# tobifinn/torch-assimilate

Hardware: AMD Instinct MI355X
Metric: local analyses/sec (LETKF, 40-member) (higher is better)
Workload: dtype f32

## Files before the change

include/mia_letkf.h:

```cpp
#ifndef MIA_LETKF_H
#define MIA_LETKF_H

#include <stddef.h>
#include <stdint.h>

#ifdef __cplusplus
extern "C" {
#endif

#define MIA_VERSION 100

#define MIA_OK 0
#define MIA_ERR_NULL (-1)
#define MIA_ERR_SIZE (-2)
#define MIA_ERR_UNSUPPORTED (-3)
#define MIA_ERR_WORKSPACE (-4)
#define MIA_ERR_ALIGN (-5)
#define MIA_ERR_COMM (-6)
#define MIA_ERR_ARG (-7)

#define MIA_FLAG_OVERFLOW 1
#define MIA_FLAG_NOCONV 2
#define MIA_FLAG_NONFINITE 4
#define MIA_FLAG_RETRY 8
// ... 355 lines not shown
                               const double* rec, int64_t P,
                               const int32_t* nbr_cnt, const int32_t* nbr_idx, const double* nbr_w, int p_cap, int p_max,
                               double epsilon, double* W_out, int32_t* flags, int32_t* retry_count, void* stream);
int mia_lienks_update_wide_f64_cover(int k, int p_max, int64_t n_points, int64_t P);
int mia_lienks_update_stream_f64(const double* W_in, int64_t w_stride, int k, int64_t g0, int64_t g1,
                                 const double* rec, int64_t P,
                                 const int32_t* nbr_cnt, const int32_t* nbr_idx, const double* nbr_w, int p_cap, int p_max,
                                 double epsilon, double* W_out, int32_t* flags, int32_t* retry_count, void* stream);
int mia_lienks_update_stream_f64_cover(int k, int p_max, int64_t n_points, int64_t P);

int mia_obs_space_uncorr_f32(const float* hx, int64_t ldh, const float* y, const float* var, int k, int64_t P,
                             float* Yb_opt, int64_t ldy, float* d_opt, float* rec_opt, void* stream);
int mia_obs_space_uncorr_f64(const double* hx, int64_t ldh, const double* y, const double* var, int k, int64_t P,
                             double* Yb_opt, int64_t ldy, double* d_opt, double* rec_opt, void* stream);
int mia_obs_space_corr_workspace_bytes(int k, int64_t P, int elem_bytes, size_t* bytes);
int mia_obs_space_corr_f32(const float* hx, int64_t ldh, const float* y, const float* cov, int k, int64_t P,
                           float* Yb_opt, int64_t ldy, float* d_opt, float* rec_opt, int32_t* info_opt,
                           void* ws, size_t ws_bytes, void* stream);
int mia_obs_space_corr_f64(const double* hx, int64_t ldh, const double* y, const double* cov, int k, int64_t P,
                           double* Yb_opt, int64_t ldy, double* d_opt, double* rec_opt, int32_t* info_opt,
                           void* ws, size_t ws_bytes, void* stream);

typedef struct mia_comm mia_comm_t;
typedef int (*mia_allgather_fn)(void* ctx, const void* send, void* recv, size_t bytes_per_rank, void* stream);
typedef int (*mia_allreduce_max_i32_fn)(void* ctx, int32_t* buf, int n, void* stream);
int mia_comm_load(const char* rccl_library_path );
int mia_comm_unique_id(void* id128);
int mia_comm_create(const void* id128, int rank, int world, mia_comm_t** comm);
int mia_comm_create_partition(int rank, int world, mia_comm_t** out);
int mia_comm_create_custom(int rank, int world, mia_allgather_fn allgather, mia_allreduce_max_i32_fn allreduce_max,
                           void* ctx, mia_comm_t** comm);
int mia_letkf_step_submit(const float* X, int64_t G, int m, int k, const float* Yb, const float* d, int64_t P,
                          const double* grid_xyz, const double* obs_xyz, int n_coord, const int32_t* coord_group,
                          const double* gc_c, int n_r, double gc_eps, float inf_factor, float gamma, int method,
                          int p_max_assumed, mia_comm_t* comm, int n_chunks, int phase, float* Xa, int32_t* flags,
                          int32_t* counters, void* ws, size_t ws_bytes, void* stream, void* comm_stream, void* prep_stream,
                          int step_flags, int32_t* host8, void* after_stream, void* on_stream, void** done_event,
                          void* time_start_event, void* time_stop_event, void** job_out);
int mia_letkf_step_join(void* job);
typedef struct mia_step_args {
  const float* X; int64_t G; int32_t m, k; const float* Yb; const float* d; int64_t P;
  const double* grid_xyz; const double* obs_xyz; int32_t n_coord; int32_t coord_group[MIA_MAX_COORD];
  double gc_c[MIA_MAX_RADII]; int32_t n_r; double gc_eps; float inf_factor, gamma; int32_t method, p_max_assumed;
  mia_comm_t* comm; int32_t n_chunks, phase; float* Xa; int32_t* flags; int32_t* counters; void* ws; size_t ws_bytes;
  void* stream; void* comm_stream; void* prep_stream; int32_t step_flags; int32_t* host8; void* after_stream; void* on_stream;
  void** done_event; void* time_start_event; void* time_stop_event;
  void* caller_stream; void** in_event;
  double period[MIA_MAX_COORD];
} mia_step_args_t;
int mia_letkf_step_submit_args(const mia_step_args_t* a, void** job_out);
int mia_letkf_sharded_step_periodic_f32(const float* X, int64_t G, int m, int k, const float* Yb, const float* d, int64_t P,
                                        const double* grid_xyz, const double* obs_xyz, int n_coord, const int32_t* coord_group,
                                        const double* period, const double* gc_c, int n_r, double gc_eps, float inf_factor,
                                        float gamma, int method, int p_max_assumed, mia_comm_t* comm, int n_chunks, int phase,
                                        float* Xa, int32_t* flags, int32_t* counters, void* ws, size_t ws_bytes, void* stream,
                                        void* comm_stream, void* prep_stream, int step_flags);
int mia_letkf_step_run_args(const mia_step_args_t* a, int32_t* out8);
int mia_letkf_step_collect(void* job, void** done_event, const int32_t* host8, void* consumer_stream, int consumer_stream_valid,
                           int32_t* out8);
int mia_timing_event_acquire(void** event);
int mia_timing_event_release(void* event);
int mia_timing_event_elapsed_ms(void* start_event, void* stop_event, float* ms);
int mia_letkf_step_drain(void);
int mia_letkf_step_readback(const int32_t* counters, int32_t* host8, void* after_stream, void* on_stream, void** done_event);
int mia_event_synchronize(void* event);
int mia_stream_wait_event(void* stream, void* event);
int mia_stream_wait_stream(void* dst_stream, void* src_stream, void** event_io);
int mia_event_destroy(void* event);
int mia_letkf_step_launch_stats(double* prep_us, double* rest_us, long long* steps);
int mia_comm_set_place_stream(mia_comm_t* comm, void* stream);
int mia_comm_peer_alloc(mia_comm_t* comm, size_t result_bytes, int n_slots, void* ipc_handles_out);
int mia_comm_peer_open(mia_comm_t* comm, const void* all_handles);
int mia_comm_peer_attach(mia_comm_t* comm, int peer, void* const* result_bufs, void* sync_area);
int mia_comm_peer_wait_bound(mia_comm_t* comm, int log2_polls);
void* mia_comm_peer_buffer(mia_comm_t* comm, int slot);
void* mia_comm_peer_sync_area(mia_comm_t* comm);
int mia_comm_peer_exchange(mia_comm_t* comm, int slot, int rows, int64_t G, int64_t b0, int64_t b1, int32_t* counters,
                           void* stream);
int mia_comm_peer_rewait(mia_comm_t* comm, int slot, int32_t* counters, void* stream);
int mia_comm_destroy(mia_comm_t* comm);
const char* mia_comm_last_error(void);
int mia_letkf_sharded_step_workspace_bytes(int64_t G, int m, int k, int64_t P, int n_coord, int world,
                                           int n_chunks, int p_max_assumed, size_t* bytes);
int mia_letkf_step_workspace_release(void* ws);
int mia_debug_step_trace(long long* out, int max_steps);
int mia_letkf_sharded_step_f32(const float* X , int64_t G, int m, int k,
                               const float* Yb , const float* d , int64_t P,
                               const double* grid_xyz , const double* obs_xyz ,
                               int n_coord, const int32_t* coord_group , const double* gc_c ,
                               int n_r, double gc_eps, float inf_factor, float gamma, int method,
                               int p_max_assumed, mia_comm_t* comm, int n_chunks, int phase,
                               float* Xa , int32_t* flags, int32_t* counters,
                               void* ws, size_t ws_bytes, void* stream, void* comm_stream);

#define MIA_STEP_NO_JOIN 1
#define MIA_STEP_WS_CLEAN 4
#define MIA_STEP_TILE_EXTRA(n) (((n) & 7) << 4)
#define MIA_STEP_FRESH_BOX 0x400
#define MIA_STEP_SCAN_INDEX 0x800
#define MIA_STEP_REUSE_LISTS 0x1000
#define MIA_STEP_KEEP_LISTS 0x4000
#define MIA_STEP_NO_GATHER 0x2000
#define MIA_STEP_NO_TILE_LISTS 8
int mia_letkf_sharded_step_streams_f32(const float* X, int64_t G, int m, int k,
                                       const float* Yb, const float* d, int64_t P,
                                       const double* grid_xyz, const double* obs_xyz,
                                       int n_coord, const int32_t* coord_group , const double* gc_c ,
                                       int n_r, double gc_eps, float inf_factor, float gamma, int method,
                                       int p_max_assumed, mia_comm_t* comm, int n_chunks, int phase,
                                       float* Xa, int32_t* flags, int32_t* counters,
                                       void* ws, size_t ws_bytes, void* stream, void* comm_stream,
                                       void* prep_stream, int step_flags);

int mia_letkf_step_timing_events(void* start_event, void* stop_event);

#ifdef __cplusplus
}
#endif
#endif
```

torch-assimilate_amd/_cabi.py:

```python
import ctypes as C
import os

from ._build import LIB_PATH

_lib = None

i32, i64, f32, f64, vp, sz = C.c_int, C.c_int64, C.c_float, C.c_double, C.c_void_p, C.c_size_t


class KernelOp(C.Structure):
    _fields_ = [("op", C.c_int32), ("reserved", C.c_int32), ("value", C.c_double)]


_LISTS = [vp, vp, vp, i32, i32]
_SHARD = [vp, i64, i32, i32, i64, i64, vp, i64] + _LISTS


def _analysis_entry(f):
    return (_SHARD + [f, f, vp, i64, i64, vp, vp, vp], i32)


def _analysis_redo(f):
    return (_SHARD + [f, f, vp, i64, i64, vp, vp], i32)

# ... 82 lines not shown
    "mia_letkf_localize_tiles_periodic_f64": ([i32, vp, i64, i64, vp, i64, i32, C.POINTER(C.c_int32), C.POINTER(f64),
                                               C.POINTER(f64), i32, f64, i32, i32, vp, sz, vp, vp, sz, vp], i32),
    "mia_letkf_analysis_matfun_fused_f32": ([vp, i64, i32, i32, i64, i64, vp, i64, vp, i32, C.POINTER(C.c_int32),
                                             C.POINTER(f64), i32, f64, vp, sz, i32, f32, f32, vp, i64, i64, vp, vp, vp,
                                             vp], i32),
    "mia_letkf_tile_lists_bytes": ([i64, i32, i32, C.POINTER(sz)], i32),
    "mia_letkf_localize_tiles_f64": ([i32, vp, i64, i64, vp, i64, i32, C.POINTER(C.c_int32), C.POINTER(f64), i32, f64,
                                      i32, i32, vp, sz, vp, vp, sz, vp], i32),
    "mia_letkf_split_record_bytes": ([i32, C.POINTER(sz)], i32),
    "mia_letkf_pack_split_f32": ([vp, vp, i32, i64, vp, vp], i32),
    "mia_letkf_analysis_tiles_f32": ([vp, i64, i32, i32, i64, i64, vp, i64, vp, i32, i32, f32, vp, i64, i64, vp, vp, vp], i32),
    "mia_letkf_tiles_cover": ([i32, i32, i32, i32, i64, i64, i64, i64, f32], i32),
    "mia_lketkf_rbf_analysis_tiles_f32": ([vp, i64, i32, i32, i64, i64, vp, vp, i64, vp, i32, i32, f32, f32, vp, i64, i64,
                                           vp, vp, vp], i32),
    "mia_letkf_weights_tiles_f32": ([vp, i64, i32, i32, i64, i64, vp, i64, vp, i32, i32, f32, vp, i64, i64, vp, vp, vp, vp], i32),
    "mia_letkf_analysis_retry_f32": _analysis_redo(f32),
    "mia_lketkf_rbf_analysis_f32": ([vp, i64, i32, i32, i64, i64, vp, vp, i64, vp, vp, vp, i32, i32, f32, f32,
                                     vp, i64, i64, vp, vp, vp, sz, vp], i32),
    "mia_lketkf_rbf_analysis_f64": ([vp, i64, i32, i32, i64, i64, vp, vp, i64, vp, vp, vp, i32, i32, f64, f64,
                                     vp, i64, i64, vp, vp, vp, sz, vp], i32),
    "mia_etkf_workspace_bytes": ([i32, i64, i32, C.POINTER(sz)], i32),
    "mia_etkf_weights_f32": ([vp, vp, i32, i64, f32, vp, vp, vp, sz, vp], i32),
    "mia_etkf_weights_f64": ([vp, vp, i32, i64, f64, vp, vp, vp, sz, vp], i32),
    "mia_ketkf_workspace_bytes": ([i32, i64, i32, C.POINTER(sz)], i32),
    "mia_ketkf_weights_f32": ([vp, vp, i32, i64, f32, C.POINTER(KernelOp), i32, vp, vp, vp, sz, vp], i32),
    "mia_ketkf_weights_f64": ([vp, vp, i32, i64, f64, C.POINTER(KernelOp), i32, vp, vp, vp, sz, vp], i32),
    "mia_apply_weights_f32": ([vp, i64, i32, i32, i64, i64, vp, vp, i64, i64, vp], i32),
    "mia_apply_weights_f64": ([vp, i64, i32, i32, i64, i64, vp, vp, i64, i64, vp], i32),
    "mia_apply_f64_cover": ([i32, i32, i64, i64, i64], i32),
    "mia_apply_local_f64_cover": ([i32, i32, i64, i64, i64], i32),
    "mia_apply_local_weights_f32": ([vp, i64, i32, i32, i64, i64, vp, vp, i64, i64, vp], i32),
    "mia_apply_local_weights_f64": ([vp, i64, i32, i32, i64, i64, vp, vp, i64, i64, vp], i32),
    "mia_lienks_update_f32": ([vp, i64, i32, i64, i64, vp, i64, vp, vp, vp, i32, i32, f32, f32, vp, vp, vp], i32),
    "mia_lienks_update_f64": ([vp, i64, i32, i64, i64, vp, i64, vp, vp, vp, i32, i32, f64, f64, vp, vp, vp], i32),
    "mia_lienks_update_matfun_f32": _ienks_tile_entry(f32),
    "mia_lienks_update_retry_f32": ([vp, i64, i32, i64, i64, vp, i64, vp, vp, vp, i32, i32, f32, f32, vp, vp, vp], i32),
    "mia_lienks_update_matfun_f64": _ienks_tile_entry(f64),
    "mia_lienks_update_retry_f64": ([vp, i64, i32, i64, i64, vp, i64, vp, vp, vp, i32, i32, f64, f64, vp, vp, vp], i32),
    "mia_lienks_update_f64_cover": _COVER4,
    "mia_lienks_update_wide_f64": _ienks_tile_entry(f64),
    "mia_lienks_update_wide_f64_cover": _COVER4,
    "mia_lienks_update_stream_f64": _ienks_tile_entry(f64),
    "mia_lienks_update_stream_f64_cover": _COVER4,
    "mia_obs_space_uncorr_f32": ([vp, i64, vp, vp, i32, i64, vp, i64, vp, vp, vp], i32),
    "mia_obs_space_uncorr_f64": ([vp, i64, vp, vp, i32, i64, vp, i64, vp, vp, vp], i32),
    "mia_obs_space_corr_workspace_bytes": ([i32, i64, i32, C.POINTER(sz)], i32),
    "mia_obs_space_corr_f32": ([vp, i64, vp, vp, i32, i64, vp, i64, vp, vp, vp, vp, sz, vp], i32),
    "mia_obs_space_corr_f64": ([vp, i64, vp, vp, i32, i64, vp, i64, vp, vp, vp, vp, sz, vp], i32),
    "mia_comm_load": ([C.c_char_p], i32),
    "mia_comm_unique_id": ([vp], i32),
    "mia_comm_create": ([vp, i32, i32, C.POINTER(vp)], i32),
    "mia_comm_create_partition": ([i32, i32, C.POINTER(vp)], i32),
    "mia_comm_create_custom": ([i32, i32, vp, vp, vp, C.POINTER(vp)], i32),
    "mia_comm_set_place_stream": ([vp, vp], i32),
    "mia_letkf_step_submit": ([vp, i64, i32, i32, vp, vp, i64, vp, vp, i32, C.POINTER(C.c_int32), C.POINTER(f64), i32, f64,
                               f32, f32, i32, i32, vp, i32, i32, vp, vp, vp, vp, sz, vp, vp, vp, i32,
                               vp, vp, vp, C.POINTER(vp), vp, vp, C.POINTER(vp)], i32),
    "mia_letkf_step_submit_args": ([vp, vp], i32),
    "mia_letkf_step_run_args": ([vp, vp], i32),
    "mia_letkf_step_collect": ([vp, vp, vp, vp, i32, vp], i32),
    "mia_timing_event_acquire": ([C.POINTER(vp)], i32),
    "mia_timing_event_release": ([vp], i32),
    "mia_timing_event_elapsed_ms": ([vp, vp, C.POINTER(C.c_float)], i32),
    "mia_letkf_step_join": ([vp], i32),
    "mia_debug_step_trace": ([C.POINTER(C.c_longlong), i32], i32),
    "mia_letkf_step_drain": ([], i32),
    "mia_letkf_step_readback": ([vp, vp, vp, vp, C.POINTER(vp)], i32),
    "mia_event_synchronize": ([vp], i32),
    "mia_stream_wait_event": ([vp, vp], i32),
    "mia_stream_wait_stream": ([vp, vp, C.POINTER(vp)], i32),
    "mia_event_destroy": ([vp], i32),
    "mia_letkf_step_launch_stats": ([C.POINTER(C.c_double), C.POINTER(C.c_double), C.POINTER(C.c_longlong)], i32),
    "mia_comm_peer_alloc": ([vp, sz, i32, vp], i32),
    "mia_comm_peer_open": ([vp, vp], i32),
    "mia_comm_peer_attach": ([vp, i32, C.POINTER(vp), vp], i32),
    "mia_comm_peer_wait_bound": ([vp, i32], i32),
    "mia_comm_peer_buffer": ([vp, i32], vp),
    "mia_comm_peer_sync_area": ([vp], vp),
    "mia_comm_peer_exchange": ([vp, i32, i32, i64, i64, i64, vp, vp], i32),
    "mia_comm_peer_rewait": ([vp, i32, vp, vp], i32),
    "mia_comm_destroy": ([vp], i32),
    "mia_comm_last_error": ([], C.c_char_p),
    "mia_letkf_sharded_step_workspace_bytes": ([i64, i32, i32, i64, i32, i32, i32, i32, C.POINTER(sz)], i32),
    "mia_letkf_step_workspace_release": ([vp], i32),
    "mia_letkf_sharded_step_f32": ([vp, i64, i32, i32, vp, vp, i64, vp, vp, i32, C.POINTER(C.c_int32), C.POINTER(f64),
                                    i32, f64, f32, f32, i32, i32, vp, i32, i32, vp, vp, vp, vp, sz, vp, vp], i32),
    "mia_letkf_step_timing_events": ([vp, vp], i32),
    "mia_letkf_sharded_step_streams_f32": ([vp, i64, i32, i32, vp, vp, i64, vp, vp, i32, C.POINTER(C.c_int32),
                                            C.POINTER(f64), i32, f64, f32, f32, i32, i32, vp, i32, i32, vp, vp, vp, vp,
                                            sz, vp, vp, vp, i32], i32),
    "mia_letkf_sharded_step_periodic_f32": ([vp, i64, i32, i32, vp, vp, i64, vp, vp, i32, C.POINTER(C.c_int32), C.POINTER(f64),
                                             C.POINTER(f64), i32, f64, f32, f32, i32, i32, vp, i32, i32, vp, vp, vp, vp,
                                             sz, vp, vp, vp, i32], i32),
}
EXPORTED_SYMBOLS = tuple(_PROTOS)
ALLGATHER_FN = C.CFUNCTYPE(C.c_int, vp, vp, vp, sz, vp)
ALLREDUCE_MAX_I32_FN = C.CFUNCTYPE(C.c_int, vp, vp, C.c_int, vp)


class MiaError(RuntimeError):
    status = None


def lib():
    global _lib
    if _lib is None:
        if not os.path.exists(LIB_PATH):
            raise MiaError(
                "HIP extension %s not found: run `python -c \"import __graft_entry__ as g; g.build()\"` "
                "(there is no CPU fallback for the LETKF hot path)" % LIB_PATH)
        import torch
        h = C.CDLL(LIB_PATH)
        for name, (args, res) in _PROTOS.items():
            fn = getattr(h, name)
            fn.argtypes, fn.restype = args, res
        _lib = h
    return _lib


def set_option(name: str, value: int) -> int:
    old = C.c_int(0)
    check(lib().mia_get_option(name.encode(), C.byref(old)), "mia_get_option(%s)" % name)
    check(lib().mia_set_option(name.encode(), int(value)), "mia_set_option(%s)" % name)
    return old.value


class StepArgs(C.Structure):
    _fields_ = [("X", C.c_void_p), ("G", C.c_int64), ("m", C.c_int32), ("k", C.c_int32), ("Yb", C.c_void_p), ("d", C.c_void_p),
                ("P", C.c_int64), ("grid_xyz", C.c_void_p), ("obs_xyz", C.c_void_p), ("n_coord", C.c_int32),
                ("coord_group", C.c_int32 * 3), ("gc_c", C.c_double * 3), ("n_r", C.c_int32), ("gc_eps", C.c_double),
                ("inf_factor", C.c_float), ("gamma", C.c_float), ("method", C.c_int32), ("p_max_assumed", C.c_int32),
                ("comm", C.c_void_p), ("n_chunks", C.c_int32), ("phase", C.c_int32), ("Xa", C.c_void_p), ("flags", C.c_void_p),
                ("counters", C.c_void_p), ("ws", C.c_void_p), ("ws_bytes", C.c_size_t), ("stream", C.c_void_p),
                ("comm_stream", C.c_void_p), ("prep_stream", C.c_void_p), ("step_flags", C.c_int32), ("host8", C.c_void_p),
                ("after_stream", C.c_void_p), ("on_stream", C.c_void_p), ("done_event", C.POINTER(C.c_void_p)),
                ("time_start_event", C.c_void_p), ("time_stop_event", C.c_void_p), ("caller_stream", C.c_void_p),
                ("in_event", C.POINTER(C.c_void_p)), ("period", C.c_double * 3)]


class TimingEvent:
    __slots__ = ("cuda_event",)
    _free = []

    def __init__(self):
        free = TimingEvent._free
        if not free:
            l = lib()
            ev = C.c_void_p()
            for _ in range(32):
                check(l.mia_timing_event_acquire(C.byref(ev)), "mia_timing_event_acquire")
                free.append(ev.value)
        self.cuda_event = free.pop()

    def elapsed_time(self, other) -> float:
        ms = C.c_float(0.0)
        check(lib().mia_timing_event_elapsed_ms(self.cuda_event, other.cuda_event, C.byref(ms)), "mia_timing_event_elapsed_ms")
        return float(ms.value)

    def __del__(self):
        try:
            if self.cuda_event:
                TimingEvent._free.append(self.cuda_event)
        except Exception:
            pass


# ... 25 lines not shown
```

torch-assimilate_amd/csrc/localize.hip:

```cpp
#include <cstdlib>
#include "mia_common.h"
#include "mia_options.h"
#include "mia_localize_dev.h"
#include "mia_pack_dev.h"
#include "mia_tiles.h"

namespace mia {


struct IndexParams {
  const double* obs;
  int64_t P;
  int nc;
  double cutoff[MIA_MAX_COORD];
  int cell_cap;
  IndexHeader* hdr;
  int* start;
  int* cursor;
  int* sorted;
  int* cell_of;
  int* rank_of;
  double* sxyz;
  unsigned nb_bbox;
  PackJob pack;
// ... 476 lines not shown
  if (!r || !w) return MIA_ERR_NULL;
  int64_t nb = (n + 255) / 256;
  if (nb > 4096) nb = 4096;
  gc_kernel<T, TAPER><<<dim3((unsigned)nb), dim3(256), 0, stream>>>(r, n, w);
  MIA_LAUNCH_CHECK();
  return MIA_OK;
}

int check_period(const double* period, int n_coord, const double** out) {
  bool cyclic = false;
  for (int c = 0; period && c < n_coord; ++c) {
    if (!(period[c] >= 0.0) || !(period[c] < __builtin_inf())) return MIA_ERR_ARG;
    cyclic = cyclic || period[c] > 0.0;
  }
  *out = cyclic ? period : nullptr;
  return MIA_OK;
}

int index_build_impl(const double* obs_xyz, int64_t P, int n_coord, const int32_t* coord_group,
                     const double* gc_c, int n_r, void* ws, size_t ws_bytes, hipStream_t stream, const PackJob* pack,
                     const ZeroJob* zero, bool header_clean, bool sort_cells, const double* period) {
  if (P < 0 || n_coord < 1 || n_coord > MIA_MAX_COORD || n_r < 1 || n_r > MIA_MAX_RADII) return MIA_ERR_SIZE;
  if (P > 2000000000LL) return MIA_ERR_UNSUPPORTED;
  if (!coord_group || !gc_c) return MIA_ERR_NULL;
  for (int c = 0; c < n_coord; ++c) if (coord_group[c] < 0 || coord_group[c] >= n_r) return MIA_ERR_SIZE;
  for (int r = 0; r < n_r; ++r) if (!(gc_c[r] > 0.0)) return MIA_ERR_SIZE;
  if (P == 0) return MIA_OK;
  if (!obs_xyz || !ws) return MIA_ERR_NULL;
  if (((uintptr_t)ws) & 255) return MIA_ERR_ALIGN;
  const IndexLayout L = index_layout(ws, P, n_coord);
  if (ws_bytes < L.bytes) return MIA_ERR_WORKSPACE;
  IndexParams ip;
  ip.obs = obs_xyz; ip.P = P; ip.nc = n_coord; ip.cell_cap = (int)L.cap;
  for (int c = 0; c < MIA_MAX_COORD; ++c) ip.cutoff[c] = c < n_coord ? 2.0 * gc_c[coord_group[c]] : 1.0;
  ip.hdr = L.hdr; ip.start = L.start; ip.cursor = L.cursor; ip.sorted = L.sorted; ip.cell_of = L.cell_of; ip.rank_of = L.rank_of;
  ip.sxyz = L.sxyz;
  ip.bucket_total = (long long)L.bucket_total; ip.bidx = L.bidx; ip.bxyz = L.bxyz;
  for (int c = 0; c < MIA_MAX_COORD; ++c) ip.period[c] = (period && c < n_coord) ? period[c] : 0.0;
  ip.periodic = period ? 1 : 0;
  void (*count_k)(IndexParams) = period ? index_count_kernel<true> : index_count_kernel<false>;
  void (*scatter_k)(IndexParams) = period ? index_scatter_kernel<true> : index_scatter_kernel<false>;
  void (*sortcell_k)(IndexParams) = period ? index_sortcell_kernel<true> : index_sortcell_kernel<false>;
  constexpr unsigned kPrepThreads = 64;
  const unsigned nbP = (unsigned)((P + kPrepThreads - 1) / kPrepThreads);
  ip.nb_bbox = nbP < 256 ? nbP : 256;
  if (!header_clean) {
    const size_t words = ((char*)ip.sorted - (char*)ip.hdr) / sizeof(uint32_t);
    const unsigned nb = (unsigned)((words + kPrepThreads * 16 - 1) / (kPrepThreads * 16));
    index_clear_kernel<<<dim3(nb < 1024 ? (nb ? nb : 1) : 1024), dim3(kPrepThreads), 0, stream>>>(
        reinterpret_cast<uint32_t*>(ip.hdr), words);
    MIA_LAUNCH_CHECK();
  }
  ip.pack = PackJob{nullptr, nullptr, nullptr, 0, 0};
  ip.zero = zero ? *zero : ZeroJob{{nullptr, nullptr, nullptr}, {0, 0, 0}};
  unsigned nb_pack = 0;
  if (pack && pack->rec) {
    if ((P + 63) / 64 > 2000000000LL) return MIA_ERR_UNSUPPORTED;
    ip.pack = *pack;
    nb_pack = (unsigned)((P + 63) / 64);
  }
  const size_t pack_lds = nb_pack ? (size_t)64 * (ip.pack.kp + 1) * sizeof(float) : 0;
  index_bbox_dims_kernel<<<dim3(ip.nb_bbox + nb_pack), dim3(kPrepThreads), pack_lds, stream>>>(ip);
  MIA_LAUNCH_CHECK();
  count_k<<<dim3(nbP), dim3(kPrepThreads), 0, stream>>>(ip);
  MIA_LAUNCH_CHECK();
  index_scan_kernel<<<dim3(1), dim3(64), 0, stream>>>(ip);
  MIA_LAUNCH_CHECK();
  ip.scatter_xyz = sort_cells ? 0 : 1;
  scatter_k<<<dim3(nbP), dim3(kPrepThreads), 0, stream>>>(ip);
  MIA_LAUNCH_CHECK();
  if (!sort_cells) return MIA_OK;
  const size_t sort_blocks = L.cap < 8192 ? (L.cap ? L.cap : 1) : 8192;
  sortcell_k<<<dim3((unsigned)sort_blocks), dim3(kPrepThreads), 0, stream>>>(ip);
  MIA_LAUNCH_CHECK();
  return MIA_OK;
}

template <bool PER>
__global__ __launch_bounds__(64) void index_bucket_kernel(IndexParams p) {
  MIA_PREP_PRIORITY();
  MIA_PREP_PRIORITY();
  extern __shared__ __attribute__((aligned(16))) float bk_lds[];
  const bool packs = p.spack.rec != nullptr;
  if (packs) pack_split_lean_request(p.spack, p.P, (int64_t)blockIdx.x, bk_lds);
  const int64_t stride = (int64_t)gridDim.x * blockDim.x;
  for (int q = 0; q < 3; ++q)
    for (int64_t i = blockIdx.x * (int64_t)blockDim.x + threadIdx.x; i < p.zero.n[q]; i += stride) p.zero.ptr[q][i] = 0;
  const int64_t j = blockIdx.x * (int64_t)blockDim.x + threadIdx.x;
  if (j < p.P) {
    IndexHeader* h = p.hdr;
    const bool grid_ok = h->magic == kIndexMagic;
    bool ok = grid_ok && h->bucket_cap > 0;
    for (int c = 0; c < p.nc; ++c) ok = ok && h->cutoff[c] == p.cutoff[c];
    if constexpr (PER)
      for (int c = 0; c < p.nc; ++c) ok = ok && h->period[c] == p.period[c];
    const int cap = h->bucket_cap;
    int id = 0;
    bool skip = false;
    double x[MIA_MAX_COORD] = {0.0, 0.0, 0.0};
    for (int c = 0; c < p.nc; ++c) {
      x[c] = p.obs[j * p.nc + c];
      double f;
      if (PER && p.period[c] > 0.0) {
        x[c] = wrap_coord(x[c], p.period[c]);
        f = floor(x[c] * h->invh[c]);
        f = f > double(h->n[c] - 1) ? double(h->n[c] - 1) : f;
      } else {
        f = floor((x[c] - h->mn[c]) * h->invh[c]);
      }
      if (!(x[c] == x[c])) { skip = true; continue; }
      if (!(f >= 0.0 && f < double(h->n[c]))) { ok = false; continue; }
      id = id * h->n[c] + int(f);
    }
    if (!ok) {
      atomicOr(&h->err, (grid_ok && cap == 0) ? kIndexErrFull : kIndexErrBox);
    } else if (!skip) {
      const int pos = atomicAdd(&p.cursor[id], 1);
      if (pos >= cap) {
        atomicOr(&h->err, kIndexErrFull);
      } else {
        const int64_t e = (int64_t)id * cap + pos;
        p.bidx[e] = int(j);
        for (int c = 0; c < p.nc; ++c) p.bxyz[e * p.nc + c] = x[c];
      }
    }
  }
  if (packs) pack_split_lean_finish(p.spack, p.P, (int64_t)blockIdx.x, bk_lds);
}

int index_bucket_build_impl(const double* obs_xyz, int64_t P, int n_coord, const int32_t* coord_group, const double* gc_c, int n_r,
                            void* ws, size_t ws_bytes, hipStream_t stream, const ZeroJob* zero, bool fresh_box,
                            const SplitPackJob* spack, int* counts, const double* period) {
  if (P <= 0 || n_coord < 1 || n_coord > MIA_MAX_COORD || n_r < 1 || n_r > MIA_MAX_RADII) return MIA_ERR_SIZE;
  if (P > 500000000LL) return MIA_ERR_UNSUPPORTED;
  if (!coord_group || !gc_c || !obs_xyz || !ws) return MIA_ERR_NULL;
  const IndexLayout L = index_layout(ws, P, n_coord);
  if (ws_bytes < L.bytes) return MIA_ERR_WORKSPACE;
  IndexParams ip;
  for (int c = 0; c < MIA_MAX_COORD; ++c) ip.period[c] = (period && c < n_coord) ? period[c] : 0.0;
  ip.periodic = period ? 1 : 0;
  void (*bucket_k)(IndexParams) = period ? index_bucket_kernel<true> : index_bucket_kernel<false>;
  ip.obs = obs_xyz; ip.P = P; ip.nc = n_coord; ip.cell_cap = (int)L.cap;
  for (int c = 0; c < MIA_MAX_COORD; ++c) ip.cutoff[c] = c < n_coord ? 2.0 * gc_c[coord_group[c]] : 1.0;
  ip.hdr = L.hdr; ip.start = L.start; ip.cursor = L.cursor; ip.sorted = L.sorted; ip.cell_of = L.cell_of; ip.rank_of = L.rank_of;
  ip.sxyz = L.sxyz;
  ip.bucket_total = (long long)L.bucket_total; ip.bidx = L.bidx; ip.bxyz = L.bxyz;
  if (counts) ip.cursor = counts;
  ip.pack = PackJob{nullptr, nullptr, nullptr, 0, 0};
  ip.zero = ZeroJob{{nullptr, nullptr, nullptr}, {0, 0, 0}};
  ip.scatter_xyz = 0;
  constexpr unsigned kPrepThreads = 64;
  const unsigned nbP = (unsigned)((P + kPrepThreads - 1) / kPrepThreads);
  ip.nb_bbox = nbP < 256 ? nbP : 256;
  if (fresh_box) {
    const size_t words = ((char*)ip.sorted - (char*)ip.hdr) / sizeof(uint32_t);
    const unsigned nb = (unsigned)((words + kPrepThreads * 16 - 1) / (kPrepThreads * 16));
    index_clear_kernel<<<dim3(nb < 1024 ? (nb ? nb : 1) : 1024), dim3(kPrepThreads), 0, stream>>>(reinterpret_cast<uint32_t*>(ip.hdr), words);
    MIA_LAUNCH_CHECK();
    index_bbox_dims_kernel<<<dim3(ip.nb_bbox), dim3(kPrepThreads), 0, stream>>>(ip);
    MIA_LAUNCH_CHECK();
  }
  ip.zero = zero ? *zero : ZeroJob{{nullptr, nullptr, nullptr}, {0, 0, 0}};
  ip.nb_main = nbP;
  ip.spack = SplitPackJob{nullptr, nullptr, nullptr, 0};
  unsigned nb = nbP;
  size_t lds = 0;
  if (spack && spack->rec) {
    ip.spack = *spack;
    nb = (unsigned)((P + 1 + 63) / 64);
    lds = split_pack_lean_lds(spack->k);
    if (lds > kMaxDynamicLds) return MIA_ERR_UNSUPPORTED;
    if (lds > 48 * 1024) MIA_HIP_TRY(hipFuncSetAttribute((const void*)bucket_k, hipFuncAttributeMaxDynamicSharedMemorySize, (int)lds));
  }
  bucket_k<<<dim3(nb), dim3(kPrepThreads), lds, stream>>>(ip);
  MIA_LAUNCH_CHECK();
  return MIA_OK;
}

int make_scan_params(ScanParams* sp, const double* grid_xyz, int64_t P, int n_coord, const int32_t* coord_group,
                     const double* gc_c, int n_r, double gc_eps, void* ws, int taper, bool bucket) {
  if (taper != MIA_TAPER_GC && taper != MIA_TAPER_GC_INF) return MIA_ERR_SIZE;
  if (n_coord < 1 || n_coord > MIA_MAX_COORD || n_r < 1 || n_r > MIA_MAX_RADII) return MIA_ERR_SIZE;
  if (!coord_group || !gc_c || !grid_xyz || !ws) return MIA_ERR_NULL;
  const IndexLayout L = index_layout(ws, P, n_coord);
  sp->grid = grid_xyz; sp->sxyz = L.sxyz; sp->hdr = L.hdr; sp->start = L.start; sp->sorted = L.sorted;
  if (bucket) { sp->sxyz = L.bxyz; sp->start = L.cursor; sp->sorted = L.bidx; }
  sp->nc = n_coord; sp->n_r = n_r;
  for (int c = 0; c < MIA_MAX_COORD; ++c) sp->group[c] = c < n_coord ? coord_group[c] : 0;
  for (int r = 0; r < MIA_MAX_RADII; ++r) { sp->inv_c[r] = r < n_r ? 1.0 / gc_c[r] : 1.0; sp->cc[r] = r < n_r ? gc_c[r] : 1.0; }
  sp->eps = gc_eps;
  sp->taper = taper;
  for (int r = 0; r < MIA_MAX_RADII; ++r) {
    sp->four_c2[r] = 4.0 * sp->cc[r] * sp->cc[r];
    sp->inv_c_f[r] = (float)sp->inv_c[r]; sp->c_f[r] = (float)sp->cc[r]; sp->inv_c2_f[r] = (float)(sp->inv_c[r] * sp->inv_c[r]);
  }
  sp->eps_f = (float)gc_eps;
  return MIA_OK;
}

int localize_impl(const double* grid_xyz, int64_t g0, int64_t g1, const double* obs_xyz, int64_t P, int n_coord,
                  const int32_t* coord_group, const double* gc_c, int n_r, double gc_eps, int p_cap,
                  int32_t* nbr_cnt, int32_t* nbr_idx, double* nbr_w, int32_t* stats, void* ws, size_t ws_bytes,
                  hipStream_t stream, const PackJob* pack, bool stats_zeroed, const ZeroJob* zero, int taper,
                  bool header_clean, bool sort_cells, const double* period) {
  if (g1 < g0 || g0 < 0 || P < 0) return MIA_ERR_SIZE;
  if (n_coord < 1 || n_coord > MIA_MAX_COORD || n_r < 1 || n_r > MIA_MAX_RADII || p_cap < 1) return MIA_ERR_SIZE;
  if (!coord_group || !gc_c || !stats) return MIA_ERR_NULL;
  for (int c = 0; c < n_coord; ++c) if (coord_group[c] < 0 || coord_group[c] >= n_r) return MIA_ERR_SIZE;
  for (int r = 0; r < n_r; ++r) if (!(gc_c[r] > 0.0)) return MIA_ERR_SIZE;
  const int64_t ng = g1 - g0;
// ... 192 lines not shown
```

torch-assimilate_amd/csrc/mia_tiles.h:

```cpp
#pragma once
#include "mia_common.h"

namespace mia {

constexpr int kTileSlack = 8;

static inline int tile_ut_for(int p_max) {
  const int ut = (p_max + kTileSlack + 15) >> 4;
  return ut < 1 ? 1 : ut;
}

struct TileListLayout { size_t hdr, idx, D, bytes; int ut; int64_t ntile; };
static inline TileListLayout tile_list_layout(int64_t ng, int ut) {
  TileListLayout L;
  L.ut = ut;
  L.ntile = (ng + 15) >> 4;
  size_t o = 0;
  L.hdr = o; o = align_up(o + (size_t)(L.ntile > 0 ? L.ntile : 1) * 16, 256);
  L.idx = o; o = align_up(o + (size_t)(L.ntile > 0 ? L.ntile : 1) * 16 * ut * sizeof(int32_t), 256);
  L.D = o; o = align_up(o + (size_t)(L.ntile > 0 ? L.ntile : 1) * ut * 1024, 256);
  L.bytes = o;
  return L;
}

// ... 174 lines not shown
  t = (unsigned)__builtin_amdgcn_update_dpp(0, (int)u, 0x124, 0xf, 0xf, false); u = u > t ? u : t;
  t = (unsigned)__builtin_amdgcn_update_dpp(0, (int)u, 0x128, 0xf, 0xf, false); u = u > t ? u : t;
  const unsigned a = (unsigned)__builtin_amdgcn_readlane((int)u, 0), b = (unsigned)__builtin_amdgcn_readlane((int)u, 16);
  const unsigned c = (unsigned)__builtin_amdgcn_readlane((int)u, 32), d = (unsigned)__builtin_amdgcn_readlane((int)u, 48);
  const unsigned ab = a > b ? a : b, cd = c > d ? c : d;
  return ab > cd ? ab : cd;
}
__device__ __forceinline__ f4w t2_mfma3(f4w acc, const h8v ah, const h8v al, const h8v bh, const h8v bl) {
  acc = __builtin_amdgcn_mfma_f32_16x16x32_f16(al, bh, acc, 0, 0, 0);
  acc = __builtin_amdgcn_mfma_f32_16x16x32_f16(ah, bl, acc, 0, 0, 0);
  return __builtin_amdgcn_mfma_f32_16x16x32_f16(ah, bh, acc, 0, 0, 0);
}
template <typename T>
__device__ __forceinline__ T t2_ld(const void* base, unsigned byte_off) {
  return *reinterpret_cast<const T*>(reinterpret_cast<const char*>(base) + byte_off);
}
typedef short s4v __attribute__((__vector_size__(4 * sizeof(short))));
__device__ __forceinline__ s4v t2_tr_read(const unsigned char* lds_addr) {
  return __builtin_amdgcn_ds_read_tr16_b64_v4i16((__attribute__((address_space(3))) s4v*)lds_addr);
}


struct SplitPackJob { const float* Yb; const float* d; unsigned char* rec; int k; };

__device__ inline void pack_split_wave(const SplitPackJob& J, int64_t P, int64_t block, float* lds) {
  const int lane = threadIdx.x & 63;
  const int k = J.k, nc8 = (k + 7) >> 3, rb = 32 * nc8 + 16;
  const int ls = (k + 1) | 1;
  float* scl = lds + 64 * ls;
  const int64_t j0 = block * 64;
  const int64_t j = j0 + lane;
  const bool real = j < P;
  const int64_t jc = real ? j : (P > 0 ? P - 1 : 0);
  const float dj = (real && P > 0) ? J.d[jc] : 0.0f;
  constexpr int kRowsInFlight = 40;
  for (int i0 = 0; i0 < k; i0 += kRowsInFlight) {
    float v[kRowsInFlight];
#pragma unroll
    for (int u = 0; u < kRowsInFlight; ++u) {
      const int i = i0 + u < k ? i0 + u : k - 1;
      v[u] = (P > 0) ? J.Yb[(int64_t)i * P + jc] : 0.0f;
    }
#pragma unroll
    for (int u = 0; u < kRowsInFlight; ++u)
      if (i0 + u < k) lds[lane * ls + i0 + u] = real ? v[u] : 0.0f;
  }
  do { asm volatile("s_waitcnt lgkmcnt(0)" ::: "memory"); __builtin_amdgcn_wave_barrier(); } while (0);
  unsigned mx = 0u;
  for (int i = 0; i < k; ++i) {
    const unsigned a = __float_as_uint(lds[lane * ls + i]) & 0x7fffffffu;
    mx = a > mx ? a : mx;
  }
  int es;
  const float sc = pow2_scale(mx, 9, &es);
  const float wd = dj * sc;
  const bool bad = mx >= 0x7f800000u || !(fabsf(wd) < 3.0e38f);
  scl[lane] = sc;
  if (j <= P) {
    const float E = bad ? __builtin_nanf("") : __uint_as_float((unsigned)(127 - es) << 23);
    *reinterpret_cast<f4w*>(J.rec + j * rb + 32 * nc8) = f4w{wd, E, 0.0f, 0.0f};
  }
  do { asm volatile("s_waitcnt lgkmcnt(0)" ::: "memory"); __builtin_amdgcn_wave_barrier(); } while (0);
  const int nvalid = P + 1 - j0 < 64 ? (int)(P + 1 - j0) : 64;
  const int nq = nvalid * nc8;
  int r = lane / nc8, c = lane - r * nc8;
  const int dr = 64 / nc8, dc = 64 - dr * nc8;
  for (int q = lane; q < nq; q += 64) {
    const float s = scl[r];
    float x[8];
#pragma unroll
    for (int i = 0; i < 8; ++i) x[i] = 8 * c + i < k ? lds[r * ls + 8 * c + i] * s : 0.0f;
    h8v hi, lo;
    split8(x, hi, lo);
    unsigned char* o = J.rec + (j0 + r) * rb + 32 * c;
    *reinterpret_cast<h8v*>(o) = hi;
    *reinterpret_cast<h8v*>(o + 16) = lo;
    r += dr; c += dc;
    if (c >= nc8) { c -= nc8; ++r; }
  }
}

static inline size_t split_pack_lds(int k) { return ((size_t)64 * ((k + 1) | 1) + 64) * sizeof(float); }

__device__ __forceinline__ void pack_split_lean_request(const SplitPackJob& J, int64_t P, int64_t block, float* lds) {
  const int lane = threadIdx.x & 63;
  const int64_t j = block * 64 + lane;
  const int64_t jc = j < P ? j : (P > 0 ? P - 1 : 0);
  if (P > 0)
    for (int i = 0; i < J.k; ++i)
      __builtin_amdgcn_global_load_lds(reinterpret_cast<const unsigned*>(J.Yb + (int64_t)i * P + jc),
                                       (__attribute__((address_space(3))) void*)(lds + i * 64), 4, 0, 0);
}
__device__ __forceinline__ void pack_split_lean_finish(const SplitPackJob& J, int64_t P, int64_t block, const float* lds) {
  const int lane = threadIdx.x & 63;
  const int k = J.k, nc8 = (k + 7) >> 3, rb = 32 * nc8 + 16;
  const int64_t j = block * 64 + lane;
  const bool real = j < P;
  const float dj = (real && P > 0) ? J.d[j] : 0.0f;
  asm volatile("s_waitcnt vmcnt(0)" ::: "memory");
  __builtin_amdgcn_wave_barrier();
  unsigned mx = 0u;
  if (real)
    for (int i = 0; i < k; ++i) {
      const unsigned a = __float_as_uint(lds[i * 64 + lane]) & 0x7fffffffu;
      mx = a > mx ? a : mx;
    }
  int es;
  const float sc = pow2_scale(mx, 9, &es);
  const float wd = dj * sc;
  const bool bad = mx >= 0x7f800000u || !(fabsf(wd) < 3.0e38f);
  if (j > P) return;
  unsigned char* o = J.rec + j * rb;
  const float E = bad ? __builtin_nanf("") : __uint_as_float((unsigned)(127 - es) << 23);
  *reinterpret_cast<f4w*>(o + 32 * nc8) = f4w{wd, E, 0.0f, 0.0f};
  for (int c = 0; c < nc8; ++c) {
    float x[8];
#pragma unroll
    for (int i = 0; i < 8; ++i) x[i] = (real && 8 * c + i < k) ? lds[(8 * c + i) * 64 + lane] * sc : 0.0f;
    h8v hi, lo;
    split8(x, hi, lo);
    *reinterpret_cast<h8v*>(o + 32 * c) = hi;
    *reinterpret_cast<h8v*>(o + 32 * c + 16) = lo;
  }
}
static inline size_t split_pack_lean_lds(int k) { return (size_t)64 * k * sizeof(float); }

struct ScanParams;
int split_pack_launch(const float* Yb, const float* d, int k, int64_t P, void* rec, hipStream_t stream);
int tile_lists_launch(const double* grid_xyz, int64_t g0, int64_t ng, int64_t P, int n_coord, const int32_t* coord_group,
                      const double* gc_c, int n_r, double gc_eps, int taper, int ut, void* tile_lists, int32_t* stats,
                      void* index_ws, hipStream_t stream, const SplitPackJob* pack, bool bucket = false, const int* counts = nullptr,
                      const double* period = nullptr);
struct Tile2Params {
  const float* X; int64_t ldx; int m, k;
  int64_t g0, ng;
  const unsigned char* rec; int rb, nc8; int64_t zero_rec;
  const int4* thdr; const int32_t* tidx; const f4w* tD;
  float inv_reg, f0, inv_k, cs_phi, cs_psi;
  float* Xa; int64_t ldo, o0; int32_t* flags; int32_t* retry_count;
  int dmax;
  const int2* tab_hdr; const float2* tab_c;
  int seg_len; int64_t seg_stride;
  int* clr_counts; const int* clr_n; unsigned* clr_err; int32_t* err_out;
  int stagger;
};
struct Tile2Housekeeping { int* counts; const int* n; unsigned* err; int32_t* err_out; };
bool tile2_covers(int m, int k, int p_max, int extra_blocks, int64_t ldx, int64_t ldo, int64_t ng);
bool tile2_records_addressable(int k, int64_t P);
int tile2_analysis_launch(const float* X, int64_t ldx, int m, int k, int64_t g0, int64_t ng, const void* rec, int64_t P,
                          const void* tile_lists, int ut, float inf_factor, float* Xa, int64_t ldo, int64_t o0,
                          int32_t* flags, int32_t* retry_count, int dmax, const int2* tab_hdr, const float2* tab_c,
                          hipStream_t stream, int seg_len = 0, int64_t seg_stride = 0, const Tile2Housekeeping* hk = nullptr,
                          const struct Tile2Loc* loc = nullptr);
bool tile2f_covers(int m, int k, int ut, int n_coord);
int tile2f_launch(const Tile2Params& tp, const struct Tile2Loc& loc, int ut, int kt, hipStream_t stream);
size_t tile2_lds_bytes(int ut, int k);

int tile2p_launch_any(const Tile2Params& tp, int ut, int kt, hipStream_t stream);
bool lketkf_tile_covers(int m, int k, int p_max, int extra_blocks, int64_t ldx, int64_t ldo, int64_t ng, int64_t P);
int lketkf_tile_launch(const float* X, int64_t ldx, int m, int k, int64_t g0, int64_t ng, const float* Yb, const float* d,
                       int64_t P, const void* tile_lists, int ut, float inf_factor, float gamma, float* Xa, int64_t ldo,
                       int64_t o0, int32_t* flags, int32_t* retry_count, int dmax, const int2* tab_hdr, const float2* tab_c,
                       hipStream_t stream, int seg_len = 0, int64_t seg_stride = 0, const Tile2Housekeeping* hk = nullptr);

}
```

torch-assimilate_amd/csrc/sharded_step.hip:

```cpp
#include <array>
#include <atomic>
#include <chrono>
#include <condition_variable>
#include <deque>
#include <mutex>
#include <thread>
#include <vector>
#include <string.h>
#include <stdio.h>
#include <stdlib.h>

#include "mia_common.h"
#include "mia_kernels.h"
#include "mia_options.h"
#include "mia_pack_dev.h"
#include "mia_step_comm.h"
#include "mia_tiles.h"

using mia::kMaxChunks;

namespace {

struct StepLayout {
  size_t rec, loc, cnt, idx, w, done, bufs, gath, total;
// ... 128 lines not shown

static bool count_arrays_clean_for_scan(void* ws) {
  std::lock_guard<std::mutex> lock(g_stamp_mu);
  for (auto& x : g_stamps)
    if (x.ws == ws) {
      const bool clean = x.cnt_cur == 0 && !x.unknown;
      x.cnt_cur = 0;
      x.unknown = false;
      return clean;
    }
  return false;
}

extern "C" int mia_letkf_step_readback(const int32_t* counters, int32_t* host8, void* after_stream, void* on_stream,
                                       void** done_event) {
  if (!counters || !host8 || !done_event) return MIA_ERR_NULL;
  (void)hipGetLastError();
  hipStream_t a = (hipStream_t)after_stream, o = (hipStream_t)on_stream;
  hipEvent_t ev = (hipEvent_t)*done_event;
  if (!ev) {
    MIA_HIP_TRY(hipEventCreateWithFlags(&ev, hipEventDisableTiming));
    *done_event = (void*)ev;
  }
  if (a != o) {
    hipEvent_t pe;
    int rc = prep_event(&pe);
    if (rc != MIA_OK) return rc;
    MIA_HIP_TRY(hipEventRecord(pe, a));
    MIA_HIP_TRY(hipStreamWaitEvent(o, pe, 0));
  }
  MIA_HIP_TRY(hipMemcpyAsync(host8, counters, 8 * sizeof(int32_t), hipMemcpyDeviceToHost, o));
  MIA_HIP_TRY(hipEventRecord(ev, o));
  return MIA_OK;
}
static int readback_after_event(const int32_t* counters, int32_t* host8, hipEvent_t after, void* on_stream, void** done_event) {
  if (!counters || !host8 || !done_event || !after) return MIA_ERR_NULL;
  (void)hipGetLastError();
  hipStream_t o = (hipStream_t)on_stream;
  hipEvent_t ev = (hipEvent_t)*done_event;
  if (!ev) {
    MIA_HIP_TRY(hipEventCreateWithFlags(&ev, hipEventDisableTiming));
    *done_event = (void*)ev;
  }
  MIA_HIP_TRY(hipStreamWaitEvent(o, after, 0));
  MIA_HIP_TRY(hipMemcpyAsync(host8, counters, 8 * sizeof(int32_t), hipMemcpyDeviceToHost, o));
  MIA_HIP_TRY(hipEventRecord(ev, o));
  return MIA_OK;
}
extern "C" int mia_event_synchronize(void* event) {
  if (!event) return MIA_ERR_NULL;
  MIA_HIP_TRY(hipEventSynchronize((hipEvent_t)event));
  return MIA_OK;
}
extern "C" int mia_stream_wait_stream(void* dst_stream, void* src_stream, void** event_io) {
  if (!event_io) return MIA_ERR_NULL;
  (void)hipGetLastError();
  if (!*event_io) {
    hipEvent_t e = nullptr;
    MIA_HIP_TRY(hipEventCreateWithFlags(&e, hipEventDisableTiming));
    *event_io = (void*)e;
  }
  MIA_HIP_TRY(hipEventRecord((hipEvent_t)*event_io, (hipStream_t)src_stream));
  MIA_HIP_TRY(hipStreamWaitEvent((hipStream_t)dst_stream, (hipEvent_t)*event_io, 0));
  return MIA_OK;
}

extern "C" int mia_stream_wait_event(void* stream, void* event) {
  if (!event) return MIA_ERR_NULL;
  MIA_HIP_TRY(hipStreamWaitEvent((hipStream_t)stream, (hipEvent_t)event, 0));
  return MIA_OK;
}
extern "C" int mia_event_destroy(void* event) {
  if (event) (void)hipEventDestroy((hipEvent_t)event);
  return MIA_OK;
}

extern "C" int mia_letkf_sharded_step_workspace_bytes(int64_t G, int m, int k, int64_t P, int n_coord, int world,
                                                      int n_chunks, int p_max_assumed, size_t* bytes) {
  if (!bytes) return MIA_ERR_NULL;
  StepLayout L;
  int rc = step_layout(G, m, k, P, n_coord, world, n_chunks, p_max_assumed, &L);
  if (rc != MIA_OK) return rc;
  *bytes = L.total;
  return MIA_OK;
}

extern "C" int mia_letkf_sharded_step_f32(const float* X, int64_t G, int m, int k,
                                          const float* Yb, const float* d, int64_t P,
                                          const double* grid_xyz, const double* obs_xyz, int n_coord,
                                          const int32_t* coord_group, const double* gc_c, int n_r, double gc_eps,
                                          float inf_factor, float gamma, int method, int p_max_assumed,
                                          mia_comm_t* comm, int n_chunks, int phase,
                                          float* Xa, int32_t* flags, int32_t* counters,
                                          void* ws, size_t ws_bytes, void* stream, void* comm_stream) {
  return mia_letkf_sharded_step_streams_f32(X, G, m, k, Yb, d, P, grid_xyz, obs_xyz, n_coord, coord_group, gc_c, n_r,
                                            gc_eps, inf_factor, gamma, method, p_max_assumed, comm, n_chunks, phase, Xa,
                                            flags, counters, ws, ws_bytes, stream, comm_stream, nullptr, 0);
}

constexpr int kStepPrepDone = 0x100;

struct StepState {
  int stage = 0;
  int flags = 0;
  hipEvent_t pe = nullptr;
  uint32_t seq = 0;
  hipEvent_t kdone = nullptr;
  StepDecision dec;
};

static inline bool step_tables_fit(int n_coord, int n_r) {
  return n_coord >= 1 && n_coord <= MIA_MAX_COORD && n_r >= 1 && n_r <= MIA_MAX_RADII;
}
static inline int step_period(const mia_step_args_t& a, const double** period) {
  const int n = a.n_coord >= 1 && a.n_coord <= MIA_MAX_COORD ? a.n_coord : 0;
  return mia::check_period(a.period, n, period) != MIA_OK ? MIA_ERR_ARG : MIA_OK;
}

struct StepPlan {
  StepLayout L;
  int flags;
  int world, rank, n_chunks;
  int peer_slot, extra, pm_tl, rows;
  bool no_gather, peer, exch;
  bool signal_mode;
  bool lazy, tl_route, tl_rbf, tl_bucket, want_fused, eig_only;
  int64_t b0, b1;
  hipStream_t s, cs, ps;
  const double* period;
  const int2* tl_th;
  const float2* tl_tc;
  GeomStamp stamp;
  char* base;
  float* rec;
  int32_t *cnt, *idx, *done, *ctr;
  double* w;
  size_t gath_stride, done_ints;
  bool tl_reuse, tl_fused, cnt_must_clear, zero_in_kernel, carried;
  int* tl_counts;
  mia::Tile2Housekeeping tl_hk;
  const mia::Tile2Housekeeping* hk;
  mia::Tile2Loc tl_loc;
  const mia::Tile2Loc* loc;
};

static int step_plan(const mia_step_args_t& a, const StepState& st, StepPlan* plan) {
  StepPlan& p = *plan;
  if (step_period(a, &p.period) != MIA_OK) return MIA_ERR_ARG;
  if (!a.X || !a.Xa || !a.flags || !a.counters || !a.ws || !a.grid_xyz) return MIA_ERR_NULL;
  if (a.P > 0 && (!a.Yb || !a.d || !a.obs_xyz)) return MIA_ERR_NULL;
  if (a.method < 0 || a.method > 2 || (a.phase != 0 && a.phase != 1)) return MIA_ERR_SIZE;
  if ((uintptr_t)a.ws % 256) return MIA_ERR_ALIGN;
  if (!step_tables_fit(a.n_coord, a.n_r)) return MIA_ERR_SIZE;
  mia_comm* comm = a.comm;
  const int m = a.m, k = a.k, flags = p.flags = st.flags;
  const int64_t G = a.G, P = a.P;
  p.world = comm ? comm->world : 1;
  p.rank = comm ? comm->rank : 0;
  p.n_chunks = comm ? a.n_chunks : 1;
  p.no_gather = comm && (flags & MIA_STEP_NO_GATHER) != 0;
  if (p.no_gather) p.n_chunks = 1;
  if (comm && !p.no_gather && p.world > 1 && !comm->nccl && !comm->ag) return MIA_ERR_COMM;
  p.peer_slot = (comm && p.world > 1 && !p.no_gather) ? mia::peer_slot_of(comm, a.Xa) : -1;
  p.peer = p.peer_slot >= 0;
  if (p.peer) p.n_chunks = 1;
  p.exch = comm && !p.peer && !p.no_gather && (p.world > 1 || p.n_chunks > 1);
// ... 699 lines not shown
```

Before: 2.587 billion.

## Vectorize split-pack Yb loads and stage records in LDS for coalesced stores

```diff
diff --git a/include/mia_letkf.h b/include/mia_letkf.h
--- a/include/mia_letkf.h
+++ b/include/mia_letkf.h
@@ -461,6 +461,8 @@
 const char* mia_comm_last_error(void);
 int mia_letkf_sharded_step_workspace_bytes(int64_t G, int m, int k, int64_t P, int n_coord, int world,
                                            int n_chunks, int p_max_assumed, size_t* bytes);
+int mia_letkf_step_split_records(const void* ws, int64_t G, int m, int k, int64_t P, int n_coord, int world, int n_chunks,
+                                 int p_max_assumed, void* out, size_t out_bytes, void* stream);
 int mia_letkf_step_workspace_release(void* ws);
 int mia_debug_step_trace(long long* out, int max_steps);
 int mia_letkf_sharded_step_f32(const float* X , int64_t G, int m, int k,
diff --git a/torch-assimilate_amd/_cabi.py b/torch-assimilate_amd/_cabi.py
--- a/torch-assimilate_amd/_cabi.py
+++ b/torch-assimilate_amd/_cabi.py
@@ -188,6 +188,7 @@
     "mia_comm_destroy": ([vp], i32),
     "mia_comm_last_error": ([], C.c_char_p),
     "mia_letkf_sharded_step_workspace_bytes": ([i64, i32, i32, i64, i32, i32, i32, i32, C.POINTER(sz)], i32),
+    "mia_letkf_step_split_records": ([vp, i64, i32, i32, i64, i32, i32, i32, i32, vp, sz, vp], i32),
     "mia_letkf_step_workspace_release": ([vp], i32),
     "mia_letkf_sharded_step_f32": ([vp, i64, i32, i32, vp, vp, i64, vp, vp, i32, C.POINTER(C.c_int32), C.POINTER(f64),
                                     i32, f64, f32, f32, i32, i32, vp, i32, i32, vp, vp, vp, vp, sz, vp, vp], i32),
diff --git a/torch-assimilate_amd/csrc/localize.hip b/torch-assimilate_amd/csrc/localize.hip
--- a/torch-assimilate_amd/csrc/localize.hip
+++ b/torch-assimilate_amd/csrc/localize.hip
@@ -582,7 +582,7 @@
   MIA_PREP_PRIORITY();
   extern __shared__ __attribute__((aligned(16))) float bk_lds[];
   const bool packs = p.spack.rec != nullptr;
-  if (packs) pack_split_lean_request(p.spack, p.P, (int64_t)blockIdx.x, bk_lds);
+  const float pk_d = packs ? pack_split_lean_request(p.spack, p.P, (int64_t)blockIdx.x, bk_lds) : 0.0f;
   const int64_t stride = (int64_t)gridDim.x * blockDim.x;
   for (int q = 0; q < 3; ++q)
     for (int64_t i = blockIdx.x * (int64_t)blockDim.x + threadIdx.x; i < p.zero.n[q]; i += stride) p.zero.ptr[q][i] = 0;
@@ -625,7 +625,7 @@
       }
     }
   }
-  if (packs) pack_split_lean_finish(p.spack, p.P, (int64_t)blockIdx.x, bk_lds);
+  if (packs) pack_split_lean_finish(p.spack, p.P, (int64_t)blockIdx.x, bk_lds, pk_d);
 }
 
 int index_bucket_build_impl(const double* obs_xyz, int64_t P, int n_coord, const int32_t* coord_group, const double* gc_c, int n_r,
diff --git a/torch-assimilate_amd/csrc/mia_tiles.h b/torch-assimilate_amd/csrc/mia_tiles.h
--- a/torch-assimilate_amd/csrc/mia_tiles.h
+++ b/torch-assimilate_amd/csrc/mia_tiles.h
@@ -280,21 +280,30 @@
 
 static inline size_t split_pack_lds(int k) { return ((size_t)64 * ((k + 1) | 1) + 64) * sizeof(float); }
 
-__device__ __forceinline__ void pack_split_lean_request(const SplitPackJob& J, int64_t P, int64_t block, float* lds) {
+__device__ __forceinline__ float pack_split_lean_request(const SplitPackJob& J, int64_t P, int64_t block, float* lds) {
   const int lane = threadIdx.x & 63;
-  const int64_t j = block * 64 + lane;
+  const int k = J.k;
+  const int64_t j0 = block * 64, j = j0 + lane;
   const int64_t jc = j < P ? j : (P > 0 ? P - 1 : 0);
-  if (P > 0)
-    for (int i = 0; i < J.k; ++i)
-      __builtin_amdgcn_global_load_lds(reinterpret_cast<const unsigned*>(J.Yb + (int64_t)i * P + jc),
-                                       (__attribute__((address_space(3))) void*)(lds + i * 64), 4, 0, 0);
-}
-__device__ __forceinline__ void pack_split_lean_finish(const SplitPackJob& J, int64_t P, int64_t block, const float* lds) {
+  if (P <= 0) return 0.0f;
+  int i = 0;
+  if ((reinterpret_cast<uintptr_t>(J.Yb) & 15) == 0 && (P & 3) == 0 && j0 + 64 <= P) {
+    const float* src = J.Yb + (int64_t)(lane >> 4) * P + j0 + 4 * (lane & 15);
+    for (; i + 4 <= k; i += 4)
+      __builtin_amdgcn_global_load_lds(reinterpret_cast<const unsigned*>(src + (int64_t)i * P),
+                                       (__attribute__((address_space(3))) void*)(lds + i * 64), 16, 0, 0);
+  }
+  for (; i < k; ++i)
+    __builtin_amdgcn_global_load_lds(reinterpret_cast<const unsigned*>(J.Yb + (int64_t)i * P + jc),
+                                     (__attribute__((address_space(3))) void*)(lds + i * 64), 4, 0, 0);
+  return j < P ? J.d[j] : 0.0f;
+}
+__device__ __forceinline__ void pack_split_lean_finish(const SplitPackJob& J, int64_t P, int64_t block, float* lds, const float dj) {
   const int lane = threadIdx.x & 63;
   const int k = J.k, nc8 = (k + 7) >> 3, rb = 32 * nc8 + 16;
-  const int64_t j = block * 64 + lane;
+  const int64_t j0 = block * 64, j = j0 + lane;
   const bool real = j < P;
-  const float dj = (real && P > 0) ? J.d[j] : 0.0f;
+  unsigned char* img = reinterpret_cast<unsigned char*>(lds);
   asm volatile("s_waitcnt vmcnt(0)" ::: "memory");
   __builtin_amdgcn_wave_barrier();
   unsigned mx = 0u;
@@ -307,21 +316,49 @@
   const float sc = pow2_scale(mx, 9, &es);
   const float wd = dj * sc;
   const bool bad = mx >= 0x7f800000u || !(fabsf(wd) < 3.0e38f);
-  if (j > P) return;
-  unsigned char* o = J.rec + j * rb;
   const float E = bad ? __builtin_nanf("") : __uint_as_float((unsigned)(127 - es) << 23);
-  *reinterpret_cast<f4w*>(o + 32 * nc8) = f4w{wd, E, 0.0f, 0.0f};
   for (int c = 0; c < nc8; ++c) {
     float x[8];
 #pragma unroll
-    for (int i = 0; i < 8; ++i) x[i] = (real && 8 * c + i < k) ? lds[(8 * c + i) * 64 + lane] * sc : 0.0f;
+    for (int i = 0; i < 8; ++i) x[i] = lds[(8 * c + i) * 64 + lane];
+#pragma unroll
+    for (int i = 0; i < 8; ++i) x[i] = (real && 8 * c + i < k) ? x[i] * sc : 0.0f;
     h8v hi, lo;
     split8(x, hi, lo);
-    *reinterpret_cast<h8v*>(o + 32 * c) = hi;
-    *reinterpret_cast<h8v*>(o + 32 * c + 16) = lo;
-  }
-}
-static inline size_t split_pack_lean_lds(int k) { return (size_t)64 * k * sizeof(float); }
+    unsigned char* o = img + c * 2048 + ((lane ^ (c & 7)) << 5);
+    *reinterpret_cast<h8v*>(o) = hi;
+    *reinterpret_cast<h8v*>(o + 16) = lo;
+  }
+  do { asm volatile("s_waitcnt lgkmcnt(0)" ::: "memory"); __builtin_amdgcn_wave_barrier(); } while (0);
+  const int npr = 2 * nc8 + 1;
+  const int nvalid = P + 1 - j0 < 64 ? (int)(P + 1 - j0) : 64;
+  const int np = nvalid * npr;
+  const int dr = 64 / npr, dp = 64 - dr * npr;
+  int r = lane / npr, p = lane - r * npr;
+  unsigned char* o = J.rec + j0 * rb + lane * 16;
+  constexpr int kPieces = 3;
+  for (int t0 = 0; t0 < np; t0 += 64 * kPieces) {
+    f4w v[kPieces];
+#pragma unroll
+    for (int u = 0; u < kPieces; ++u) {
+      const int c = p >> 1;
+      const bool tail = p == 2 * nc8;
+      int off = c * 2048 + ((r ^ (c & 7)) << 5) + ((p & 1) << 4);
+      off = (!tail && t0 + 64 * u + lane < np) ? off : 0;
+      v[u] = *reinterpret_cast<const f4w*>(img + off);
+      const float wd_r = __int_as_float(__builtin_amdgcn_ds_bpermute(r << 2, __float_as_int(wd)));
+      const float E_r = __int_as_float(__builtin_amdgcn_ds_bpermute(r << 2, __float_as_int(E)));
+      if (tail) v[u] = f4w{wd_r, E_r, 0.0f, 0.0f};
+      r += dr; p += dp;
+      if (p >= npr) { p -= npr; ++r; }
+    }
+#pragma unroll
+    for (int u = 0; u < kPieces; ++u)
+      if (t0 + 64 * u + lane < np) *reinterpret_cast<f4w*>(o + 1024 * u) = v[u];
+    o += 1024 * kPieces;
+  }
+}
+static inline size_t split_pack_lean_lds(int k) { return (size_t)((k + 7) >> 3) * 2048; }
 
 struct ScanParams;
 int split_pack_launch(const float* Yb, const float* d, int k, int64_t P, void* rec, hipStream_t stream);
diff --git a/torch-assimilate_amd/csrc/sharded_step.hip b/torch-assimilate_amd/csrc/sharded_step.hip
--- a/torch-assimilate_amd/csrc/sharded_step.hip
+++ b/torch-assimilate_amd/csrc/sharded_step.hip
@@ -234,6 +234,19 @@
   int rc = step_layout(G, m, k, P, n_coord, world, n_chunks, p_max_assumed, &L);
   if (rc != MIA_OK) return rc;
   *bytes = L.total;
+  return MIA_OK;
+}
+
+extern "C" int mia_letkf_step_split_records(const void* ws, int64_t G, int m, int k, int64_t P, int n_coord, int world, int n_chunks,
+                                            int p_max_assumed, void* out, size_t out_bytes, void* stream) {
+  if (!ws || !out) return MIA_ERR_NULL;
+  StepLayout L;
+  int rc = step_layout(G, m, k, P, n_coord, world, n_chunks, p_max_assumed, &L);
+  if (rc != MIA_OK) return rc;
+  if (L.tl == L.hrec) return MIA_ERR_UNSUPPORTED;
+  const size_t bytes = (size_t)(P + 1) * mia::split_rec_bytes(k);
+  if (out_bytes < bytes) return MIA_ERR_WORKSPACE;
+  MIA_HIP_TRY(hipMemcpyAsync(out, (const char*)ws + L.hrec, bytes, hipMemcpyDefault, (hipStream_t)stream));
   return MIA_OK;
 }
 
```

New measurement: 2.744 billion (median of 5 runs). +6.1%, better.
